# CycloneBoy/pdf_table

Hardware: AMD Instinct MI355X
Metric: pages/s (higher is better)
Workload: dtype bf16

## Files before the change

pdf_table_amd/csrc/det_kernels.hip:

```cpp
#include <math.h>

#include "common.h"

namespace PT_FMT_NS {

typedef __attribute__((ext_vector_type(4))) uint32_t u32x4;
typedef __attribute__((ext_vector_type(2))) uint32_t u32x2;

__device__ __forceinline__ float bf2f(uint32_t bits16) { return a16_to_f32(bits16); }
__device__ __forceinline__ uint32_t f2bf(float f) { return f32_to_a16(f); }

struct ResizeCoef {
  int s0, s1;
  int a0, a1;
};
__device__ __forceinline__ ResizeCoef resize_coef(int d, double scale, int ssize, bool clamp_frac) {
  float f = (float)(((double)d + 0.5) * scale - 0.5);
  int s = (int)floorf(f);
  f -= (float)s;
  ResizeCoef c;
  if (clamp_frac) {
    if (s < 0) { f = 0.f; s = 0; }
    if (s >= ssize - 1) { f = 0.f; s = ssize - 1; }
  }
// ... 43 lines not shown
      const int y = blockIdx.y * PRE_ROWS + ry;
      if (y >= nh) break;
      const long long i = ((long long)b * nh + y) * nw + x;
      int v[3];
      if (w == nw && h == nh) {
        const uint8_t* p = src + ((size_t)y * w + x) * 3;
        v[0] = p[0]; v[1] = p[1]; v[2] = p[2];
      } else if (area2) {
        const uint8_t* p0 = src + ((size_t)(2 * y) * w + 2 * x) * 3;
        const uint8_t* p1 = p0 + (size_t)w * 3;
#pragma unroll
        for (int c = 0; c < 3; ++c) v[c] = (p0[c] + p0[3 + c] + p1[c] + p1[3 + c] + 2) >> 2;
      } else {
        const ResizeCoef cy = resize_coef(y, sy, h, false);
        const uint8_t* r0 = src + (size_t)cy.s0 * w * 3;
        const uint8_t* r1 = src + (size_t)cy.s1 * w * 3;
        unsigned long long q0, q1;
        if (o0 + 8 <= w * 3) {
          __builtin_memcpy(&q0, r0 + o0, 8);
          __builtin_memcpy(&q1, r1 + o0, 8);
        } else {
          q0 = q1 = 0;
          for (int k = 0; k < 3; ++k) {
            q0 |= (unsigned long long)r0[o0 + k] << (8 * k) | (unsigned long long)r0[cx.s1 * 3 + k] << (d1 + 8 * k);
            q1 |= (unsigned long long)r1[o0 + k] << (8 * k) | (unsigned long long)r1[cx.s1 * 3 + k] << (d1 + 8 * k);
          }
        }
#pragma unroll
        for (int c = 0; c < 3; ++c) {
          const int S0 = (int)((q0 >> (8 * c)) & 0xFF) * cx.a0 + (int)((q0 >> (d1 + 8 * c)) & 0xFF) * cx.a1;
          const int S1 = (int)((q1 >> (8 * c)) & 0xFF) * cx.a0 + (int)((q1 >> (d1 + 8 * c)) & 0xFF) * cx.a1;
          v[c] = (((cy.a0 * (S0 >> 4)) >> 16) + ((cy.a1 * (S1 >> 4)) >> 16) + 2) >> 2;
          v[c] = v[c] < 0 ? 0 : (v[c] > 255 ? 255 : v[c]);
        }
      }
      const uint32_t e0 = lut[0][v[2]], e1 = lut[1][v[1]], e2 = lut[2][v[0]];
      if (!split) {
        u32x2 pk;
        pk.x = (e0 & 0xFFFFu) | (e1 << 16);
        pk.y = e2 & 0xFFFFu;
        *reinterpret_cast<u32x2*>(out + (size_t)i * 4) = pk;
      } else {
        u32x4 pk;
        pk.x = (e0 & 0xFFFFu) | (e1 << 16);
        pk.y = e2 & 0xFFFFu;
        pk.z = (e0 >> 16) | (e1 & 0xFFFF0000u);
        pk.w = e2 >> 16;
        *reinterpret_cast<u32x4*>(out + (size_t)i * 8) = pk;
      }
    }
  }
}

int pt_launch_det_preprocess(const uint8_t* pages, int n, int h, int w, int nh, int nw, int flavour, int split,
                             bf16_t* out, hipStream_t s) {
  PT_REQUIRE(n > 0 && nh > 0 && nw > 0 && nh < 65536 && n < 65536, "det pre-process: bad extents %d x %d x %d", n, nh, nw);
  hipLaunchKernelGGL(det_preprocess_kernel, dim3((nw + 255) / 256, (nh + PRE_ROWS - 1) / PRE_ROWS, n), dim3(256), 0, s, pages, n, h, w, nh, nw, flavour, split, out,
                     (double)w / nw, (double)h / nh);
  PT_HIP_CHECK(hipGetLastError());
  return PT_OK;
}

__device__ __forceinline__ uint32_t bfmax2(uint32_t a, uint32_t b) {
  const float al = a16lo_f32(a), bl = a16lo_f32(b);
  const float ah = a16hi_f32(a), bh = a16hi_f32(b);
  const uint32_t lo = (bl > al) ? (b & 0xFFFFu) : (a & 0xFFFFu);
  const uint32_t hi = (bh > ah) ? (b & 0xFFFF0000u) : (a & 0xFFFF0000u);
  return lo | hi;
}

__global__ __launch_bounds__(256) void maxpool3x3s2_split_kernel(const bf16_t* __restrict__ in, int B, int H, int W,
                                                                  int C, bf16_t* __restrict__ out) {
  a16_kernel_enter();
  const int Ho = (H + 2 - 3) / 2 + 1, Wo = (W + 2 - 3) / 2 + 1;
  const int cg = C >> 3;
  const long long total = (long long)B * Ho * Wo * cg;
  for (long long i = (long long)blockIdx.x * blockDim.x + threadIdx.x; i < total; i += (long long)gridDim.x * blockDim.x) {
    const int g = (int)(i % cg);
    long long t = i / cg;
    const int ox = (int)(t % Wo);
    t /= Wo;
    const int oy = (int)(t % Ho);
    const int b = (int)(t / Ho);
    uint32_t bh[8], bl[8];
    float bv[8];
    bool first = true;
    for (int dy = 0; dy < 3; ++dy) {
      const int iy = oy * 2 - 1 + dy;
      if ((unsigned)iy >= (unsigned)H) continue;
      for (int dx = 0; dx < 3; ++dx) {
        const int ix = ox * 2 - 1 + dx;
        if ((unsigned)ix >= (unsigned)W) continue;
        const bf16_t* px = in + (((size_t)b * H + iy) * W + ix) * (2 * C) + g * 8;
        const u32x4 vh = *reinterpret_cast<const u32x4*>(px);
        const u32x4 vl = *reinterpret_cast<const u32x4*>(px + C);
        const uint32_t hw[4] = {vh.x, vh.y, vh.z, vh.w}, lw[4] = {vl.x, vl.y, vl.z, vl.w};
#pragma unroll
        for (int k = 0; k < 8; ++k) {
          const uint32_t hb = (k & 1) ? (hw[k >> 1] >> 16) : (hw[k >> 1] & 0xFFFFu);
          const uint32_t lb = (k & 1) ? (lw[k >> 1] >> 16) : (lw[k >> 1] & 0xFFFFu);
          const float v = bf2f(hb) + bf2f(lb);
          if (first || v > bv[k]) { bv[k] = v; bh[k] = hb; bl[k] = lb; }
        }
        first = false;
      }
    }
    u32x4 oh, ol;
    oh.x = bh[0] | (bh[1] << 16); oh.y = bh[2] | (bh[3] << 16); oh.z = bh[4] | (bh[5] << 16); oh.w = bh[6] | (bh[7] << 16);
    ol.x = bl[0] | (bl[1] << 16); ol.y = bl[2] | (bl[3] << 16); ol.z = bl[4] | (bl[5] << 16); ol.w = bl[6] | (bl[7] << 16);
// ... 465 lines not shown
```

pdf_table_amd/csrc/lore_kernels.hip:

```cpp
#include <stdio.h>
#include <stdlib.h>

#include "common.h"

namespace PT_FMT_NS {

typedef __attribute__((ext_vector_type(4))) uint32_t u32x4;
typedef __attribute__((ext_vector_type(2))) uint32_t u32x2;

namespace {

__device__ __forceinline__ float bf2f(uint32_t b) { return a16_to_f32(b); }
__device__ __forceinline__ uint32_t f2bf(float f) { return f32_to_a16(f); }

__device__ __forceinline__ void load8(const bf16_t* p, int lo_off, int split, float* v) {
  const u32x4 h = *reinterpret_cast<const u32x4*>(p);
  const uint32_t hw[4] = {h.x, h.y, h.z, h.w};
#pragma unroll
  for (int k = 0; k < 8; ++k) v[k] = bf2f((k & 1) ? (hw[k >> 1] >> 16) : (hw[k >> 1] & 0xFFFFu));
  if (split) {
    const u32x4 l = *reinterpret_cast<const u32x4*>(p + lo_off);
    const uint32_t lw[4] = {l.x, l.y, l.z, l.w};
#pragma unroll
    for (int k = 0; k < 8; ++k) v[k] += bf2f((k & 1) ? (lw[k >> 1] >> 16) : (lw[k >> 1] & 0xFFFFu));
// ... 230 lines not shown
        else
          store8(out + oo, C, PACKED == 1 ? 0 : split, acc);
      }
  }
}

__global__ __launch_bounds__(256) void tsr_preprocess_kernel(const uint8_t* __restrict__ pages, int ph, int pw,
                                                              const pt_tsr_table* __restrict__ tabs, int H, int W, int bgr,
                                                              const float* __restrict__ lut, bf16_t* __restrict__ out,
                                                              int split) {
  a16_kernel_enter();
  const int t = blockIdx.y;
  const int i = blockIdx.x * blockDim.x + threadIdx.x;
  if (i >= H * W) return;
  const int y = i / W, x = i - y * W;
  const pt_tsr_table tb = tabs[t];
  auto sat = [](double v) { return (long long)fmin(fmax(rint(v), -2147483648.0), 2147483647.0); };
  const long long adelta = sat(tb.minv[0] * x * 1024.0), bdelta = sat(tb.minv[3] * x * 1024.0);
  const long long X0 = sat((tb.minv[1] * y + tb.minv[2]) * 1024.0) + 16, Y0 = sat((tb.minv[4] * y + tb.minv[5]) * 1024.0) + 16;
  const long long X = (X0 + adelta) >> 5, Y = (Y0 + bdelta) >> 5;
  long long sx = X >> 5, sy = Y >> 5;
  sx = sx < -32768 ? -32768 : (sx > 32767 ? 32767 : sx);
  sy = sy < -32768 ? -32768 : (sy > 32767 ? 32767 : sy);
  const int ax = (int)(X & 31), ay = (int)(Y & 31);
  const int wt[4] = {(32 - ay) * (32 - ax) * 32, (32 - ay) * ax * 32, ay * (32 - ax) * 32, ay * ax * 32};
  int acc[3] = {0, 0, 0};
  const uint8_t* pg = pages + (size_t)tb.page * ph * pw * 3;
#pragma unroll
  for (int k = 0; k < 4; ++k) {
    const long long yy = sy + (k >> 1), xx = sx + (k & 1);
    if (yy < 0 || yy >= tb.crop_h || xx < 0 || xx >= tb.crop_w) continue;
    const long long py = tb.y0 + yy, px = tb.x0 + xx;
    if (py < 0 || py >= ph || px < 0 || px >= pw) continue;
    const uint8_t* s = pg + ((size_t)py * pw + px) * 3;
    acc[0] += s[0] * wt[k]; acc[1] += s[1] * wt[k]; acc[2] += s[2] * wt[k];
  }
  float v[3];
#pragma unroll
  for (int c = 0; c < 3; ++c) {
    const int sc = bgr ? 2 - c : c;
    int u = (acc[sc] + (1 << 14)) >> 15;
    u = u < 0 ? 0 : (u > 255 ? 255 : u);
    v[c] = lut[c * 256 + u];
  }
  bf16_t* o = out + ((size_t)t * H * W + i) * (split ? 8 : 4);
  uint32_t hb[3];
#pragma unroll
  for (int c = 0; c < 3; ++c) { hb[c] = f2bf(v[c]); o[c] = (bf16_t)hb[c]; }
  o[3] = 0;
  if (split) {
#pragma unroll
    for (int c = 0; c < 3; ++c) o[4 + c] = (bf16_t)f2bf(v[c] - bf2f(hb[c]));
    o[7] = 0;
  }
}

typedef __attribute__((ext_vector_type(8))) __bf16 dbf16x8;
typedef __attribute__((ext_vector_type(16))) float df32x16;
typedef __attribute__((ext_vector_type(2))) float df2;
__device__ __forceinline__ uint32_t pack_df2(df2 v) { return pack_a16x2(v.x, v.y); }
__device__ __forceinline__ df2 unpack_df2(uint32_t pk) { return df2{a16lo_f32(pk), a16hi_f32(pk)}; }

template <int SPLIT, int NB>
__global__ __launch_bounds__(256, (SPLIT || NB > 64) ? 2 : 4) void dcn_fused_kernel(const bf16_t* __restrict__ x, const float* __restrict__ om,
                                                            const bf16_t* __restrict__ w, const float* __restrict__ bias,
                                                            bf16_t* __restrict__ out, long long npix, int H, int W, int C,
                                                            int N, int relu) {
#pragma clang fp contract(fast)
  a16_kernel_enter();
  constexpr int ROW = 80;
  constexpr int NP = SPLIT ? 2 : 1;
  constexpr int NT = NB / 32;
  __shared__ __attribute__((aligned(16))) char s_a[NP][128 * ROW];
  __shared__ __attribute__((aligned(16))) char s_w[NP][NB * ROW];
  const int tid = threadIdx.x, lane = tid & 63, wave = tid >> 6;
  const int lx = lane & 31, q = lane >> 5;
  const long long p0 = (long long)blockIdx.x * 128;
  const int n0 = blockIdx.y * NB;
  const int cs = SPLIT ? 2 * C : C;
  const int nslice = C >> 5, nk = 9 * nslice;
  const int gp = tid & 127, gh = tid >> 7;
  long long pix = p0 + gp;
  const bool live = pix < npix;
  if (!live) pix = npix - 1;
  const int xw = (int)(pix % W), yh = (int)((pix / W) % H);
  const bf16_t* xb = x + (size_t)(pix / ((long long)W * H)) * H * W * cs;
  const float* omp = om + pix * 32;
  constexpr int WPIECES = NB * 4 / 256;
  const bf16_t* wbase = w + (size_t)(n0 >> 6) * (SPLIT ? 3 : 1) * nk * (64 * 32);

  df32x16 acc[NT];
#pragma unroll
  for (int t = 0; t < NT; ++t)
#pragma unroll
    for (int r = 0; r < 16; ++r) acc[t][r] = 0.f;

  int coff[4];
  float cwt[4], mask = 0.f;
  u32x4 rc[NP][4][2];
  u32x4 rw[NP][WPIECES];

  auto geometry = [&](int tap) {
    const float off_h = omp[2 * tap], off_w = omp[2 * tap + 1];
    mask = 1.f / (1.f + expf(-omp[18 + tap]));
    const float h_im = (float)(yh - 1 + tap / 3) + off_h;
    const float w_im = (float)(xw - 1 + tap % 3) + off_w;
// ... 1399 lines not shown
  PT_HIP_CHECK(hipGetLastError());
  return PT_OK;
}

int pt_launch_dwconvt_up_add(const bf16_t* in, const float* w, const bf16_t* add, bf16_t* out, int B, int h, int wd,
                             int C, int f, int split, hipStream_t s) {
  PT_REQUIRE(in && w && out && C % 8 == 0 && (f == 2 || f == 4), "dwconvT: bad arguments");
  const long long blocks2 = (long long)B * h * wd * (C / 8);
  const char* sw = getenv("PT_DWCONVT2");
  if (f == 2 && blocks2 < (1ll << 31) && C <= 512 && !(sw && sw[0] == '0')) {
    static int packed = -1;
    if (packed < 0) {
      const char* ev = getenv("PT_DWCONVT2_PACKED");
      packed = ev ? atoi(ev) : 1;
    }
    if (!split && packed)
      hipLaunchKernelGGL(dwconvt_up2_add_kernel<1>, dim3(grid_for(blocks2)), dim3(256), (size_t)16 * C * sizeof(float), s, in, w, add, out,
                         B, h, wd, C, 0);
    else if (split && packed)
      hipLaunchKernelGGL(dwconvt_up2_add_kernel<2>, dim3(grid_for(blocks2)), dim3(256), (size_t)16 * C * sizeof(float), s, in, w, add, out,
                         B, h, wd, C, 1);
    else
      hipLaunchKernelGGL(dwconvt_up2_add_kernel<0>, dim3(grid_for(blocks2)), dim3(256), (size_t)16 * C * sizeof(float), s, in, w, add, out,
                         B, h, wd, C, split);
    PT_HIP_CHECK(hipGetLastError());
    return PT_OK;
  }
  hipLaunchKernelGGL(dwconvt_up_add_kernel, dim3(grid_for((long long)B * h * f * wd * f * (C / 8))), dim3(256), 0, s, in,
                     w, add, out, B, h, wd, C, f, split);
  PT_HIP_CHECK(hipGetLastError());
  return PT_OK;
}

int pt_launch_dwconvt_up2_slice(const bf16_t* in, const float* w, bf16_t* out, int out_cstride, int out_coff, int out_lo_off, int B,
                                int h, int wd, int C, int split, hipStream_t s) {
  PT_REQUIRE(in && w && out && C % 8 == 0 && C <= 512 && out_cstride % 8 == 0 && out_coff % 8 == 0 && out_lo_off % 8 == 0 &&
                 out_coff + C * (split ? 2 : 1) <= out_cstride && (!split || out_coff + out_lo_off + C <= out_cstride),
             "dwconvT slice: bad arguments");
  const long long blocks2 = (long long)B * h * wd * (C / 8);
  PT_REQUIRE(blocks2 < (1ll << 31), "dwconvT slice: map too large");
  if (split)
    hipLaunchKernelGGL((dwconvt_up2_add_kernel<2, true>), dim3(grid_for(blocks2)), dim3(256), (size_t)16 * C * sizeof(float), s, in, w,
                       (const bf16_t*)nullptr, out + out_coff, B, h, wd, C, 1, out_cstride, out_lo_off);
  else
    hipLaunchKernelGGL((dwconvt_up2_add_kernel<1, true>), dim3(grid_for(blocks2)), dim3(256), (size_t)16 * C * sizeof(float), s, in, w,
                       (const bf16_t*)nullptr, out + out_coff, B, h, wd, C, 0, out_cstride, 0);
  PT_HIP_CHECK(hipGetLastError());
  return PT_OK;
}

int pt_launch_tsr_preprocess(const uint8_t* pages, int ph, int pw, const pt_tsr_table* tabs, int n, int H, int W, int bgr,
                             const float* lut, bf16_t* out, int split, hipStream_t s) {
  PT_REQUIRE(pages && tabs && lut && out && n > 0 && H > 0 && W > 0, "tsr preprocess: bad arguments");
  hipLaunchKernelGGL(tsr_preprocess_kernel, dim3((H * W + 255) / 256, n), dim3(256), 0, s, pages, ph, pw, tabs, H, W, bgr, lut,
                     out, split);
  PT_HIP_CHECK(hipGetLastError());
  return PT_OK;
}

template <int SPLIT, int NB>
static int launch_dcn_fused(pt_engine* e, const bf16_t* x, const float* om, const bf16_t* w, const float* bias, bf16_t* out,
                            int B, int H, int W, int C, int N, int relu, hipStream_t s) {
  const long long npix = (long long)B * H * W;
  char label[48];
  snprintf(label, sizeof(label), "dcn fused %d->%d @%dx%d%s", C, N, H, W, SPLIT ? " x3" : "");
  PtProfScope prof(e, s, PT_PROF_OTHER, 0, label);
  hipLaunchKernelGGL((dcn_fused_kernel<SPLIT, NB>), dim3((unsigned)((npix + 127) / 128), N / NB), dim3(256), 0, s, x, om, w,
                     bias, out, npix, H, W, C, N, relu);
  PT_HIP_CHECK(hipGetLastError());
  return PT_OK;
}

bool pt_dcn_fuses_om(const pt_engine* e, int C, int split) {
  const char* ev = getenv("PT_DCN_FUSE_OM");
  const int on = ev ? atoi(ev) : 1;
  const char* nt = getenv("PT_DCN_THREADS");
  const char* ea = getenv("PT_DCN_EARLY");
  const char* xf = getenv("PT_DCN_X3_FAST");
  const bool defaults = !(nt && atoi(nt) != 512) && !(ea && atoi(ea) == 0) && !(xf && atoi(xf) == 0);
  if (!on || !e || C % 64 != 0 || !defaults || (!split && e->dcn_mfma != 0)) return false;
  return on == 2 || (!split && C <= 128);
}

bool pt_dcn_fuses_up(const pt_engine* e, int C, int N, int split) {
  const char* ev = getenv("PT_IDA_FUSE_UP");
  if ((ev && atoi(ev) == 0) || !e || split || e->dcn_mfma != 0 || C != N || (N != 64 && N != 128)) return false;
  for (const char* name : {"PT_DCN_FUSED", "PT_DCN_FUSE_OM", "PT_DCN_THREADS", "PT_DCN_EARLY", "PT_DCN_NB", "PT_DCN_MFMA", "PT_DCN_MFMA_NB", "PT_DCN_X3_FAST"})
    if (getenv(name)) return false;
  return true;
}

int pt_launch_dcn_fused(pt_engine* e, const bf16_t* x, const float* om, const bf16_t* w, const float* bias, bf16_t* out,
                        int B, int H, int W, int C, int N, int split, int relu, hipStream_t s, const bf16_t* omw, const float* omb,
                        const bf16_t* up_in, const float* up_w, int up_f) {
  PT_REQUIRE(e && x && (om || (omw && omb)) && w && bias && out && C % 32 == 0 && N % 64 == 0, "dcn fused: bad arguments (C=%d N=%d)", C, N);
  PT_REQUIRE(!omw || pt_dcn_fuses_om(e, C, split), "dcn fused: the offset conv can only be fused on the default fused64 paths (C=%d)", C);
  PT_REQUIRE((long long)H * W * (split ? 2 * C : C) < (1ll << 31), "dcn fused: image too large for 32-bit offsets");
  if (up_f) {
    PT_REQUIRE(up_in && up_w && (up_f == 2 || (up_f == 4 && N == 64)) && H % up_f == 0 && W % up_f == 0,
               "dcn fused + up: factor %d must be 2 (or 4 at 64 channels) and divide the %dx%d map", up_f, H, W);
    PT_REQUIRE(pt_dcn_fuses_up(e, C, N, split), "dcn fused + up: only the default single-pass kernels at C = N = 64 or 128 carry the up-sampling epilogue (C=%d N=%d split=%d)", C, N, split);
  }
  const double dcn_bytes = (double)B * H * W * ((split ? 2.0 : 1.0) * 2.0 * (C + N) + 27 * 4.0) + (double)N * 9 * C * 2.0 * (split ? 3 : 1) +
                           (up_f ? (double)B * (H / up_f) * (W / up_f) * N * 2.0 : 0.0);
  e->prof.next_bytes = dcn_bytes;
  static int x3fast = -1;
// ... 152 lines not shown
```

pdf_table_amd/csrc/rec_kernels.hip:

```cpp
#include <math.h>

#include "common.h"

namespace PT_FMT_NS {

typedef __attribute__((ext_vector_type(8))) __bf16 bf16x8;
typedef __attribute__((ext_vector_type(16))) float f32x16;
typedef __attribute__((ext_vector_type(4))) uint32_t u32x4;
typedef __attribute__((ext_vector_type(2))) uint32_t u32x2;

__device__ __forceinline__ float rbf2f(uint32_t bits16) { return a16_to_f32(bits16); }
__device__ __forceinline__ uint32_t rf2bf(float f) { return f32_to_a16(f); }

__global__ __launch_bounds__(256) void rec_warp_kernel(const uint8_t* __restrict__ pages, int ph, int pw,
                                                        const pt_rec_line* __restrict__ lines, int n_lines,
                                                        const long long* __restrict__ pix_off, uint8_t* __restrict__ crops) {
  a16_kernel_enter();
  const int li = blockIdx.y;
  if (li >= n_lines) return;
  const pt_rec_line L = lines[li];
  const int cw = L.crop_w, chh = L.crop_h;
  const long long npx = (long long)cw * chh;
  uint8_t* dst = crops + pix_off[li] * 3;
  const uint8_t* src = pages + (size_t)L.page * ph * pw * 3;
  for (long long i = (long long)blockIdx.x * blockDim.x + threadIdx.x; i < npx; i += (long long)gridDim.x * blockDim.x) {
    const int x = (int)(i % cw), y = (int)(i / cw);
    int v[3];
    pt_warp_sample(src, ph, pw, L.minv, x, y, v);
#pragma unroll
    for (int c = 0; c < 3; ++c) dst[i * 3 + c] = (uint8_t)v[c];
  }
}

__global__ __launch_bounds__(1024) void rec_offsets_kernel(const pt_rec_line* __restrict__ lines, int n,
                                                           long long* __restrict__ off) {
  a16_kernel_enter();
  __shared__ long long sc[1024];
  __shared__ long long carry;
  const int tid = threadIdx.x;
  if (tid == 0) { carry = 0; off[0] = 0; }
  __syncthreads();
  for (int base = 0; base < n; base += 1024) {
    const int i = base + tid;
    long long v = 0;
    if (i < n) {
      v = (long long)lines[i].crop_w * (long long)lines[i].crop_h;
      if (v < 0) v = 0;
    }
    sc[tid] = v;
    __syncthreads();
    for (int d = 1; d < 1024; d <<= 1) {
      const long long t = tid >= d ? sc[tid - d] : 0;
      __syncthreads();
      sc[tid] += t;
      __syncthreads();
    }
    if (i < n) off[i + 1] = carry + sc[tid];
    __syncthreads();
    if (tid == 1023) carry += sc[1023];
    __syncthreads();
  }
}

int pt_launch_rec_offsets(const pt_rec_line* lines, int n, long long* off, hipStream_t s) {
  hipLaunchKernelGGL(rec_offsets_kernel, dim3(1), dim3(1024), 0, s, lines, n, off);
  PT_HIP_CHECK(hipGetLastError());
  return PT_OK;
}

int pt_launch_rec_warp(const uint8_t* pages, int ph, int pw, const pt_rec_line* lines, int n_lines,
                       const long long* pix_off, uint8_t* crops, int max_crop_px, hipStream_t s) {
  if (n_lines <= 0) return PT_OK;
  int bx = (max_crop_px + 255) / 256;
  bx = bx < 1 ? 1 : (bx > 64 ? 64 : bx);
  hipLaunchKernelGGL(rec_warp_kernel, dim3(bx, n_lines), dim3(256), 0, s, pages, ph, pw, lines, n_lines, pix_off, crops);
  PT_HIP_CHECK(hipGetLastError());
  return PT_OK;
}

struct RCoef {
  int s0, s1, a0, a1;
};
__device__ __forceinline__ RCoef rcoef(int d, double scale, int ssize, bool clamp_frac) {
  float f = (float)(((double)d + 0.5) * scale - 0.5);
  int s = (int)floorf(f);
  f -= (float)s;
  if (clamp_frac) {
    if (s < 0) { f = 0.f; s = 0; }
    if (s >= ssize - 1) { f = 0.f; s = ssize - 1; }
  }
  RCoef c;
  c.a0 = (int)rintf((1.f - f) * 2048.f);
  c.a1 = (int)rintf(f * 2048.f);
  int t0 = s, t1 = s + 1;
  c.s0 = t0 < 0 ? 0 : (t0 >= ssize ? ssize - 1 : t0);
  c.s1 = t1 < 0 ? 0 : (t1 >= ssize ? ssize - 1 : t1);
  return c;
}

__global__ __launch_bounds__(256) void rec_resize_gray_kernel(const uint8_t* __restrict__ crops,
                                                               const pt_rec_line* __restrict__ lines,
                                                               const long long* __restrict__ pix_off, int n_lines, int TH,
                                                               int TWID, int split, bf16_t* __restrict__ out,
                                                               float* __restrict__ out_f32) {
  a16_kernel_enter();
  const long long total = (long long)n_lines * TH * TWID;
  for (long long i = (long long)blockIdx.x * blockDim.x + threadIdx.x; i < total; i += (long long)gridDim.x * blockDim.x) {
    const int x = (int)(i % TWID);
    const long long t = i / TWID;
    const int y = (int)(t % TH);
    const int li = (int)(t / TH);
    const int cw = lines[li].crop_w, chh = lines[li].crop_h;
    float gray = 0.f;
    if (cw > 0 && chh > 0) {
      const double ratio = (double)cw / (double)chh;
      const int nw = ratio > (double)TWID / (double)TH ? TWID : (int)((double)TH * ratio);
      if (x < nw) {
        const uint8_t* src = crops + pix_off[li] * 3;
        int v[3];
        if (cw == nw && chh == TH) {
          const uint8_t* p = src + ((size_t)y * cw + x) * 3;
          v[0] = p[0]; v[1] = p[1]; v[2] = p[2];
        } else if (cw == 2 * nw && chh == 2 * TH) {
          const uint8_t* p0 = src + ((size_t)(2 * y) * cw + 2 * x) * 3;
          const uint8_t* p1 = p0 + (size_t)cw * 3;
#pragma unroll
          for (int c = 0; c < 3; ++c) v[c] = (p0[c] + p0[3 + c] + p1[c] + p1[3 + c] + 2) >> 2;
        } else {
          const RCoef cx = rcoef(x, (double)cw / nw, cw, true);
          const RCoef cy = rcoef(y, (double)chh / TH, chh, false);
          const uint8_t* r0 = src + (size_t)cy.s0 * cw * 3;
          const uint8_t* r1 = src + (size_t)cy.s1 * cw * 3;
#pragma unroll
          for (int c = 0; c < 3; ++c) {
            const int S0 = r0[cx.s0 * 3 + c] * cx.a0 + r0[cx.s1 * 3 + c] * cx.a1;
            const int S1 = r1[cx.s0 * 3 + c] * cx.a0 + r1[cx.s1 * 3 + c] * cx.a1;
            int r = (((cy.a0 * (S0 >> 4)) >> 16) + ((cy.a1 * (S1 >> 4)) >> 16) + 2) >> 2;
            v[c] = r < 0 ? 0 : (r > 255 ? 255 : r);
          }
        }
        const float R = (float)v[0] / 255.f, G = (float)v[1] / 255.f, B = (float)v[2] / 255.f;
        gray = (R * 0.2989f + G * 0.5870f) + B * 0.1140f;
      }
    }
    if (out_f32) {
      out_f32[i] = gray;
      continue;
    }
    const uint32_t hb = rf2bf(gray);
    if (split) {
      out[i * 2] = (bf16_t)hb;
      out[i * 2 + 1] = (bf16_t)rf2bf(gray - rbf2f(hb));
    } else {
      out[i] = (bf16_t)hb;
    }
  }
}

int pt_launch_rec_resize_gray(const uint8_t* crops, const pt_rec_line* lines, const long long* pix_off, int n_lines,
                              int split, bf16_t* out, hipStream_t s) {
  if (n_lines <= 0) return PT_OK;
  const long long total = (long long)n_lines * 32 * 640;
  int blocks = (int)((total + 255) / 256);
  if (blocks > 256 * 32) blocks = 256 * 32;
  hipLaunchKernelGGL(rec_resize_gray_kernel, dim3(blocks), dim3(256), 0, s, crops, lines, pix_off, n_lines, 32, 640, split, out,
                     static_cast<float*>(nullptr));
  PT_HIP_CHECK(hipGetLastError());
  return PT_OK;
}

int pt_launch_rec_resize_gray_f32(const uint8_t* crops, const pt_rec_line* lines, const long long* pix_off, int n_lines, int tw,
                                  float* out, hipStream_t s) {
  if (n_lines <= 0) return PT_OK;
  const long long total = (long long)n_lines * 32 * tw;
  int blocks = (int)((total + 255) / 256);
  if (blocks > 256 * 32) blocks = 256 * 32;
  hipLaunchKernelGGL(rec_resize_gray_kernel, dim3(blocks), dim3(256), 0, s, crops, lines, pix_off, n_lines, 32, tw, 0,
                     static_cast<bf16_t*>(nullptr), out);
  PT_HIP_CHECK(hipGetLastError());
  return PT_OK;
}

__global__ void crnn_limits_kernel(const pt_rec_line* __restrict__ lines, int n, int* l1, int* l2a, int* l2b, int* l3a, int* l3b,
                                   int* l0, int* __restrict__ cols) {
  a16_kernel_enter();
  __shared__ int sums[6];
  if (threadIdx.x < 6) sums[threadIdx.x] = 0;
  __syncthreads();
  int acc[6] = {0, 0, 0, 0, 0, 0};
  for (int b = blockIdx.x * blockDim.x + threadIdx.x; b < n; b += gridDim.x * blockDim.x) {
    const int cw = lines[b].crop_w, chh = lines[b].crop_h;
    int nw = 0;
    if (cw > 0 && chh > 0) {
      const double ratio = (double)cw / (double)chh;
      nw = ratio > 640.0 / 32.0 ? 640 : (int)(32.0 * ratio);
    }
    const int e0 = (nw + 2) >> 1;
    const int e1 = (e0 + 2) >> 1;
    const int v[5] = {min(e0 + 1, 320), min(e1 + 1, 160), min(e1 + 2, 160), min(e1 + 3, 160), min(e1 + 4, 160)};
    l1[b] = v[0]; l2a[b] = v[1]; l2b[b] = v[2]; l3a[b] = v[3]; l3b[b] = v[4];
    l0[b] = min((v[0] + 31) / 32 * 32 + 1, 320);
    const int tw[5] = {32, 32, 32, 32, 32}, wo[5] = {320, 160, 160, 160, 160};
#pragma unroll
    for (int k = 0; k < 5; ++k) acc[k] += min(wo[k], (v[k] + tw[k] - 1) / tw[k] * tw[k]);
    acc[5] += min(160, (v[4] + 31) / 32 * 32);
  }
#pragma unroll
  for (int k = 0; k < 6; ++k) atomicAdd(&sums[k], acc[k]);
  __syncthreads();
  if (threadIdx.x < 6) atomicAdd(&cols[threadIdx.x], sums[threadIdx.x]);
}

__global__ __launch_bounds__(1024) void rows_live_list_kernel(const int* __restrict__ lim, int n, int* __restrict__ glist) {
  a16_kernel_enter();
  __shared__ int part[1024];
  const int tid = threadIdx.x, per = (n + 1023) / 1024, b0 = tid * per, b1 = min(n, b0 + per);
  int cnt = 0;
  for (int b = b0; b < b1; ++b) cnt += min(PT_REC_T / 32, (lim[b] + 31) / 32);
  part[tid] = cnt;
  __syncthreads();
  for (int off = 1; off < 1024; off <<= 1) {
    const int v = tid >= off ? part[tid - off] : 0;
    __syncthreads();
    part[tid] += v;
    __syncthreads();
  }
// ... 1856 lines not shown
```

Measured before the change: 815.3.

## Add fast preprocessing kernels for detection, TSR, rec warp and resize

Adds four new preprocessing kernels, each on by default and switchable through a PT_PRE_FAST environment variable. Detection resize batches row loads and reuses horizontal passes across rows. TSR warp caches the LUT and per-row transforms in shared memory. Rec warp switches to a flat grid over all crop pixels using binary search on the offsets, and rec resize-gray uses one block per line with per-column coefficients in shared memory and vectorized stores. These target memory traffic and load imbalance in the preprocessing stages, at the risk of small numeric differences and extra code paths.

```diff
diff --git a/pdf_table_amd/csrc/det_kernels.hip b/pdf_table_amd/csrc/det_kernels.hip
--- a/pdf_table_amd/csrc/det_kernels.hip
+++ b/pdf_table_amd/csrc/det_kernels.hip
@@ -119,9 +119,127 @@
   }
 }
 
+constexpr int PRE_FAST_ROWS = 16, PRE_FAST_BATCH = 8;
+
+__global__ __launch_bounds__(256) void det_preprocess_fast_kernel(const uint8_t* __restrict__ pages, int n, int h, int w,
+                                                                   int nh, int nw, int flavour, int split, bf16_t* __restrict__ out,
+                                                                   double sx, double sy) {
+  a16_kernel_enter();
+  __shared__ uint32_t lut[3][256];
+  __shared__ int rowc[PRE_FAST_ROWS][4];
+  {
+    const int u = threadIdx.x;
+#pragma unroll
+    for (int c = 0; c < 3; ++c) {
+      float o;
+      if (flavour == PT_DET_PRE_DB_TORCH) {
+        const float mean[3] = {123.68f, 116.78f, 103.94f};
+        o = ((float)u - mean[c]) / 255.f;
+      } else {
+        const float scale = (float)(1.0 / 255.0);
+        const float mean[3] = {0.485f, 0.456f, 0.406f};
+        const float stdv[3] = {0.229f, 0.224f, 0.225f};
+        o = ((float)u * scale - mean[c]) / stdv[c];
+      }
+      const uint32_t hi = f2bf(o);
+      lut[c][u] = hi | (f2bf(o - bf2f(hi)) << 16);
+    }
+    if (u < PRE_FAST_ROWS) {
+      const int y = min((int)blockIdx.y * PRE_FAST_ROWS + u, nh - 1);
+      const ResizeCoef cy = resize_coef(y, sy, h, false);
+      rowc[u][0] = cy.s0; rowc[u][1] = cy.s1; rowc[u][2] = cy.a0; rowc[u][3] = cy.a1;
+    }
+  }
+  __syncthreads();
+  const int x = blockIdx.x * blockDim.x + threadIdx.x;
+  if (x >= nw) return;
+  const int b = blockIdx.z;
+  const uint8_t* src = pages + (size_t)b * h * w * 3;
+  const ResizeCoef cx = resize_coef(x, sx, w, true);
+  const int o0 = cx.s0 * 3, d1 = (cx.s1 - cx.s0) * 24;
+  const bool wide = o0 + 8 <= w * 3;
+  auto bytes = [&](int row) {
+    const uint8_t* r = src + (size_t)row * w * 3;
+    unsigned long long q = 0;
+    for (int k = 0; k < 3; ++k) q |= (unsigned long long)r[o0 + k] << (8 * k) | (unsigned long long)r[cx.s1 * 3 + k] << (d1 + 8 * k);
+    return q;
+  };
+  auto hpass = [&](unsigned long long q, int S[3]) {
+    const uint32_t p0 = (uint32_t)q, p1 = d1 ? (uint32_t)(q >> 24) : p0;
+#pragma unroll
+    for (int c = 0; c < 3; ++c) S[c] = (__mul24((int)((p0 >> (8 * c)) & 0xFF), cx.a0) + __mul24((int)((p1 >> (8 * c)) & 0xFF), cx.a1)) >> 4;
+  };
+  int have = -1;
+  int H1[3] = {0, 0, 0};
+  for (int g = 0; g < PRE_FAST_ROWS; g += PRE_FAST_BATCH) {
+    if ((int)blockIdx.y * PRE_FAST_ROWS + g >= nh) break;
+    unsigned long long q0[PRE_FAST_BATCH], q1[PRE_FAST_BATCH];
+    int s0[PRE_FAST_BATCH], s1[PRE_FAST_BATCH];
+#pragma unroll
+    for (int k = 0; k < PRE_FAST_BATCH; ++k) {
+      s0[k] = __builtin_amdgcn_readfirstlane(rowc[g + k][0]);
+      s1[k] = __builtin_amdgcn_readfirstlane(rowc[g + k][1]);
+      q0[k] = q1[k] = 0;
+      if (s0[k] != (k ? s1[k - 1] : have)) {
+        if (wide) __builtin_memcpy(&q0[k], src + (size_t)s0[k] * w * 3 + o0, 8); else q0[k] = bytes(s0[k]);
+      }
+      if (s1[k] != s0[k]) {
+        if (wide) __builtin_memcpy(&q1[k], src + (size_t)s1[k] * w * 3 + o0, 8); else q1[k] = bytes(s1[k]);
+      }
+    }
+#pragma unroll
+    for (int k = 0; k < PRE_FAST_BATCH; ++k) {
+      const int y = (int)blockIdx.y * PRE_FAST_ROWS + g + k;
+      if (y >= nh) break;
+      const int a0 = __builtin_amdgcn_readfirstlane(rowc[g + k][2]), a1 = __builtin_amdgcn_readfirstlane(rowc[g + k][3]);
+      int H0[3];
+      if (s0[k] != (k ? s1[k - 1] : have)) {
+        hpass(q0[k], H0);
+      } else {
+        H0[0] = H1[0]; H0[1] = H1[1]; H0[2] = H1[2];
+      }
+      if (s1[k] != s0[k]) {
+        hpass(q1[k], H1);
+      } else {
+        H1[0] = H0[0]; H1[1] = H0[1]; H1[2] = H0[2];
+      }
+      int v[3];
+#pragma unroll
+      for (int c = 0; c < 3; ++c) {
+        v[c] = ((__mul24(a0, H0[c]) >> 16) + (__mul24(a1, H1[c]) >> 16) + 2) >> 2;
+        v[c] = v[c] < 0 ? 0 : (v[c] > 255 ? 255 : v[c]);
+      }
+      const long long i = ((long long)b * nh + y) * nw + x;
+      const uint32_t e0 = lut[0][v[2]], e1 = lut[1][v[1]], e2 = lut[2][v[0]];
+      if (!split) {
+        u32x2 pk;
+        pk.x = (e0 & 0xFFFFu) | (e1 << 16);
+        pk.y = e2 & 0xFFFFu;
+        *reinterpret_cast<u32x2*>(out + (size_t)i * 4) = pk;
+      } else {
+        u32x4 pk;
+        pk.x = (e0 & 0xFFFFu) | (e1 << 16);
+        pk.y = e2 & 0xFFFFu;
+        pk.z = (e0 >> 16) | (e1 & 0xFFFF0000u);
+        pk.w = e2 >> 16;
+        *reinterpret_cast<u32x4*>(out + (size_t)i * 8) = pk;
+      }
+    }
+    have = s1[PRE_FAST_BATCH - 1];
+  }
+}
+
 int pt_launch_det_preprocess(const uint8_t* pages, int n, int h, int w, int nh, int nw, int flavour, int split,
                              bf16_t* out, hipStream_t s) {
   PT_REQUIRE(n > 0 && nh > 0 && nw > 0 && nh < 65536 && n < 65536, "det pre-process: bad extents %d x %d x %d", n, nh, nw);
+  const char* sw = getenv("PT_PRE_FAST");
+  const bool resample = !(w == nw && h == nh) && !(w == 2 * nw && h == 2 * nh);
+  if (resample && !(sw && sw[0] == '0')) {
+    hipLaunchKernelGGL(det_preprocess_fast_kernel, dim3((nw + 255) / 256, (nh + PRE_FAST_ROWS - 1) / PRE_FAST_ROWS, n), dim3(256), 0, s, pages, n, h, w, nh,
+                       nw, flavour, split, out, (double)w / nw, (double)h / nh);
+    PT_HIP_CHECK(hipGetLastError());
+    return PT_OK;
+  }
   hipLaunchKernelGGL(det_preprocess_kernel, dim3((nw + 255) / 256, (nh + PRE_ROWS - 1) / PRE_ROWS, n), dim3(256), 0, s, pages, n, h, w, nh, nw, flavour, split, out,
                      (double)w / nw, (double)h / nh);
   PT_HIP_CHECK(hipGetLastError());
diff --git a/pdf_table_amd/csrc/lore_kernels.hip b/pdf_table_amd/csrc/lore_kernels.hip
--- a/pdf_table_amd/csrc/lore_kernels.hip
+++ b/pdf_table_amd/csrc/lore_kernels.hip
@@ -306,6 +306,100 @@
 #pragma unroll
     for (int c = 0; c < 3; ++c) o[4 + c] = (bf16_t)f2bf(v[c] - bf2f(hb[c]));
     o[7] = 0;
+  }
+}
+
+constexpr int TSR_TILE_H = 32, TSR_BATCH = 4;
+__global__ __launch_bounds__(256) void tsr_preprocess_fast_kernel(const uint8_t* __restrict__ pages, int ph, int pw,
+                                                                   const pt_tsr_table* __restrict__ tabs, int H, int W, int bgr,
+                                                                   const float* __restrict__ lut, bf16_t* __restrict__ out,
+                                                                   int split) {
+  a16_kernel_enter();
+  __shared__ uint32_t slut[3 * 256];
+  __shared__ long long rowt[TSR_TILE_H][2];
+  const int tid = threadIdx.x, t = blockIdx.z;
+  const pt_tsr_table tb = tabs[t];
+  auto sat = [](double v) { return (long long)fmin(fmax(rint(v), -2147483648.0), 2147483647.0); };
+  for (int k = tid; k < 3 * 256; k += 256) {
+    const float v = lut[k];
+    const uint32_t hb = f2bf(v);
+    slut[k] = hb | (f2bf(v - bf2f(hb)) << 16);
+  }
+  const int yb = blockIdx.y * TSR_TILE_H;
+  if (tid < TSR_TILE_H) {
+    const int y = yb + tid;
+    rowt[tid][0] = sat((tb.minv[1] * y + tb.minv[2]) * 1024.0) + 16;
+    rowt[tid][1] = sat((tb.minv[4] * y + tb.minv[5]) * 1024.0) + 16;
+  }
+  __syncthreads();
+  const int x = blockIdx.x * 64 + (tid & 63);
+  if (x >= W) return;
+  const long long adelta = sat(tb.minv[0] * x * 1024.0), bdelta = sat(tb.minv[3] * x * 1024.0);
+  const uint8_t* pg = pages + (size_t)tb.page * ph * pw * 3;
+  auto bound = [](long long v) { return (int)(v < -65536 ? -65536 : (v > 65536 ? 65536 : v)); };
+  const int xlo = bound(tb.x0 < 0 ? -(long long)tb.x0 : 0), xhi = bound((long long)pw - tb.x0 < tb.crop_w ? (long long)pw - tb.x0 : tb.crop_w);
+  const int ylo = bound(tb.y0 < 0 ? -(long long)tb.y0 : 0), yhi = bound((long long)ph - tb.y0 < tb.crop_h ? (long long)ph - tb.y0 : tb.crop_h);
+  const int last = ph * pw - 1;
+  for (int r0 = tid >> 6; r0 < TSR_TILE_H; r0 += 4 * TSR_BATCH) {
+    if (yb + r0 >= H) break;
+    uint32_t q[TSR_BATCH][4];
+    int wt[TSR_BATCH][4];
+#pragma unroll
+    for (int k = 0; k < TSR_BATCH; ++k) {
+      const int r = r0 + 4 * k;
+      const int X = (int)((rowt[r][0] + adelta) >> 5), Y = (int)((rowt[r][1] + bdelta) >> 5);
+      int sx = X >> 5, sy = Y >> 5;
+      sx = sx < -32768 ? -32768 : (sx > 32767 ? 32767 : sx);
+      sy = sy < -32768 ? -32768 : (sy > 32767 ? 32767 : sy);
+      const int ax = X & 31, ay = Y & 31;
+      const int w4[4] = {__mul24(32 - ay, 32 - ax) * 32, __mul24(32 - ay, ax) * 32, __mul24(ay, 32 - ax) * 32, __mul24(ay, ax) * 32};
+#pragma unroll
+      for (int j = 0; j < 4; ++j) {
+        const int yy = sy + (j >> 1), xx = sx + (j & 1);
+        wt[k][j] = (yy >= ylo && yy < yhi && xx >= xlo && xx < xhi) ? w4[j] : 0;
+        const long long pyl = (long long)tb.y0 + yy, pxl = (long long)tb.x0 + xx;
+        const int py = (int)(pyl < 0 ? 0 : (pyl > ph - 1 ? ph - 1 : pyl)), px = (int)(pxl < 0 ? 0 : (pxl > pw - 1 ? pw - 1 : pxl));
+        const int pi = __mul24(py, pw) + px;
+        const int adj = pi == last ? 1 : 0;
+        uint32_t v;
+        __builtin_memcpy(&v, pg + (pi * 3 - adj), 4);
+        q[k][j] = v >> (8 * adj);
+      }
+    }
+#pragma unroll
+    for (int k = 0; k < TSR_BATCH; ++k) {
+      const int y = yb + r0 + 4 * k;
+      if (y >= H) break;
+      int acc[3] = {0, 0, 0};
+#pragma unroll
+      for (int j = 0; j < 4; ++j) {
+        acc[0] += __mul24((int)(q[k][j] & 0xFF), wt[k][j]);
+        acc[1] += __mul24((int)((q[k][j] >> 8) & 0xFF), wt[k][j]);
+        acc[2] += __mul24((int)((q[k][j] >> 16) & 0xFF), wt[k][j]);
+      }
+      uint32_t e[3];
+#pragma unroll
+      for (int c = 0; c < 3; ++c) {
+        const int sc = bgr ? 2 - c : c;
+        int u = (acc[sc] + (1 << 14)) >> 15;
+        u = u < 0 ? 0 : (u > 255 ? 255 : u);
+        e[c] = slut[c * 256 + u];
+      }
+      const size_t i = (size_t)t * H * W + (size_t)y * W + x;
+      if (!split) {
+        u32x2 pk;
+        pk.x = (e[0] & 0xFFFFu) | (e[1] << 16);
+        pk.y = e[2] & 0xFFFFu;
+        *reinterpret_cast<u32x2*>(out + i * 4) = pk;
+      } else {
+        u32x4 pk;
+        pk.x = (e[0] & 0xFFFFu) | (e[1] << 16);
+        pk.y = e[2] & 0xFFFFu;
+        pk.z = (e[0] >> 16) | (e[1] & 0xFFFF0000u);
+        pk.w = e[2] >> 16;
+        *reinterpret_cast<u32x4*>(out + i * 8) = pk;
+      }
+    }
   }
 }
 
@@ -1811,6 +1905,14 @@
 int pt_launch_tsr_preprocess(const uint8_t* pages, int ph, int pw, const pt_tsr_table* tabs, int n, int H, int W, int bgr,
                              const float* lut, bf16_t* out, int split, hipStream_t s) {
   PT_REQUIRE(pages && tabs && lut && out && n > 0 && H > 0 && W > 0, "tsr preprocess: bad arguments");
+  const char* sw = getenv("PT_PRE_FAST");
+  if (!(sw && sw[0] == '0') && n < 65536 && (H + TSR_TILE_H - 1) / TSR_TILE_H < 65536 && ph > 0 && pw > 0 && ph < (1 << 23) && pw < (1 << 23) && (long long)ph * pw >= 2 &&
+      (long long)ph * pw * 3 < (1ll << 31)) {
+    hipLaunchKernelGGL(tsr_preprocess_fast_kernel, dim3((W + 63) / 64, (H + TSR_TILE_H - 1) / TSR_TILE_H, n), dim3(256), 0, s, pages, ph, pw, tabs, H, W,
+                       bgr, lut, out, split);
+    PT_HIP_CHECK(hipGetLastError());
+    return PT_OK;
+  }
   hipLaunchKernelGGL(tsr_preprocess_kernel, dim3((H * W + 255) / 256, n), dim3(256), 0, s, pages, ph, pw, tabs, H, W, bgr, lut,
                      out, split);
   PT_HIP_CHECK(hipGetLastError());
diff --git a/pdf_table_amd/csrc/rec_kernels.hip b/pdf_table_amd/csrc/rec_kernels.hip
--- a/pdf_table_amd/csrc/rec_kernels.hip
+++ b/pdf_table_amd/csrc/rec_kernels.hip
@@ -32,6 +32,87 @@
   }
 }
 
+__device__ __forceinline__ void warp_sample32(const uint8_t* __restrict__ src, int ph, int pw, const double* m, bool use_winv, double winv, int x, int y,
+                                              int v[3]) {
+  const double X0 = m[0] * x + m[1] * y + m[2];
+  const double Y0 = m[3] * x + m[4] * y + m[5];
+  double W = winv;
+  if (!use_winv) {
+    W = m[6] * x + m[7] * y + m[8];
+    W = W != 0. ? 32. / W : 0.;
+  }
+  const double fX = fmax(-2147483648., fmin(2147483647., X0 * W));
+  const double fY = fmax(-2147483648., fmin(2147483647., Y0 * W));
+  const int Xi = (int)rint(fX), Yi = (int)rint(fY);
+  const int sx = Xi >> 5, sy = Yi >> 5;
+  const int ax = Xi & 31, ay = Yi & 31;
+  const int w00 = __mul24(32 - ay, 32 - ax) * 32, w01 = __mul24(32 - ay, ax) * 32, w10 = __mul24(ay, 32 - ax) * 32, w11 = __mul24(ay, ax) * 32;
+  int acc[3] = {0, 0, 0};
+  auto tap = [&](int yy, int xx, int wgt) {
+    if (wgt && yy >= 0 && yy < ph && xx >= 0 && xx < pw) {
+      const uint8_t* p = src + ((size_t)yy * pw + xx) * 3;
+      acc[0] += __mul24(p[0], wgt); acc[1] += __mul24(p[1], wgt); acc[2] += __mul24(p[2], wgt);
+    }
+  };
+  tap(sy, sx, w00); tap(sy, sx + 1, w01); tap(sy + 1, sx, w10); tap(sy + 1, sx + 1, w11);
+#pragma unroll
+  for (int c = 0; c < 3; ++c) {
+    const int t = (acc[c] + (1 << 14)) >> 15;
+    v[c] = t < 0 ? 0 : (t > 255 ? 255 : t);
+  }
+}
+
+constexpr int WARP_FLAT_BLOCKS = 2048;
+
+__global__ __launch_bounds__(256) void rec_warp_fast_kernel(const uint8_t* __restrict__ pages, int ph, int pw,
+                                                             const pt_rec_line* __restrict__ lines, int n_lines,
+                                                             const long long* __restrict__ pix_off, uint8_t* __restrict__ crops) {
+  a16_kernel_enter();
+  const long long total = pix_off[n_lines];
+  long long chunk = (total + gridDim.x - 1) / gridDim.x;
+  chunk = (chunk + 255) & ~255ll;
+  const long long beg = (long long)blockIdx.x * chunk;
+  const long long end = beg + chunk < total ? beg + chunk : total;
+  long long p = beg + threadIdx.x;
+  if (p >= end) return;
+  int li = 0;
+  for (int hi = n_lines; hi - li > 1;) {
+    const int mid = (li + hi) >> 1;
+    if (pix_off[mid] <= p) li = mid; else hi = mid;
+  }
+  while (p < end) {
+    while (pix_off[li + 1] <= p) ++li;
+    const long long base = pix_off[li], next = pix_off[li + 1];
+    const long long stop = next < end ? next : end;
+    const pt_rec_line L = lines[li];
+    const int cw = L.crop_w;
+    const uint8_t* src = pages + (size_t)L.page * ph * pw * 3;
+    const bool use_winv = L.minv[6] == 0. && L.minv[7] == 0.;
+    const double winv = L.minv[8] != 0. ? 32. / L.minv[8] : 0.;
+    if (next - base > 0x7FFFFFFFll || cw <= 0) {
+      for (; p < stop; p += 256) {
+        const long long i = p - base;
+        int v[3];
+        warp_sample32(src, ph, pw, L.minv, use_winv, winv, (int)(i % cw), (int)(i / cw), v);
+        uint8_t* o = crops + p * 3;
+        o[0] = (uint8_t)v[0]; o[1] = (uint8_t)v[1]; o[2] = (uint8_t)v[2];
+      }
+      continue;
+    }
+    const uint32_t ucw = (uint32_t)cw, i0 = (uint32_t)(p - base);
+    const uint32_t dy = 256u / ucw, dx = 256u - dy * ucw;
+    uint32_t y = i0 / ucw, x = i0 - y * ucw;
+    for (; p < stop; p += 256) {
+      int v[3];
+      warp_sample32(src, ph, pw, L.minv, use_winv, winv, (int)x, (int)y, v);
+      uint8_t* o = crops + p * 3;
+      o[0] = (uint8_t)v[0]; o[1] = (uint8_t)v[1]; o[2] = (uint8_t)v[2];
+      x += dx; y += dy;
+      if (x >= ucw) { x -= ucw; ++y; }
+    }
+  }
+}
+
 __global__ __launch_bounds__(1024) void rec_offsets_kernel(const pt_rec_line* __restrict__ lines, int n,
                                                            long long* __restrict__ off) {
   a16_kernel_enter();
@@ -68,12 +149,20 @@
   return PT_OK;
 }
 
+static bool pre_fast() {
+  const char* sw = getenv("PT_PRE_FAST");
+  return !(sw && sw[0] == '0');
+}
+
 int pt_launch_rec_warp(const uint8_t* pages, int ph, int pw, const pt_rec_line* lines, int n_lines,
                        const long long* pix_off, uint8_t* crops, int max_crop_px, hipStream_t s) {
   if (n_lines <= 0) return PT_OK;
   int bx = (max_crop_px + 255) / 256;
   bx = bx < 1 ? 1 : (bx > 64 ? 64 : bx);
-  hipLaunchKernelGGL(rec_warp_kernel, dim3(bx, n_lines), dim3(256), 0, s, pages, ph, pw, lines, n_lines, pix_off, crops);
+  if (pre_fast())
+    hipLaunchKernelGGL(rec_warp_fast_kernel, dim3(WARP_FLAT_BLOCKS), dim3(256), 0, s, pages, ph, pw, lines, n_lines, pix_off, crops);
+  else
+    hipLaunchKernelGGL(rec_warp_kernel,dim3(bx, n_lines), dim3(256), 0, s, pages, ph, pw, lines, n_lines, pix_off, crops);
   PT_HIP_CHECK(hipGetLastError());
   return PT_OK;
 }
@@ -157,9 +246,120 @@
   }
 }
 
+constexpr int RG_ROWS = 16, RG_MAXW = 1024;
+
+__global__ __launch_bounds__(256) void rec_resize_gray_fast_kernel(const uint8_t* __restrict__ crops,
+                                                                    const pt_rec_line* __restrict__ lines,
+                                                                    const long long* __restrict__ pix_off, int n_lines, int TH,
+                                                                    int TWID, int split, bf16_t* __restrict__ out,
+                                                                    float* __restrict__ out_f32) {
+  a16_kernel_enter();
+  __shared__ float q255[256];
+  __shared__ int cxs[RG_MAXW];
+  __shared__ uint32_t cxa[RG_MAXW];
+  __shared__ int cys[RG_ROWS][4];
+  const int tid = threadIdx.x, li = blockIdx.x;
+  const int yb = blockIdx.y * RG_ROWS, rows = min(RG_ROWS, TH - yb);
+  const int cw = lines[li].crop_w, chh = lines[li].crop_h;
+  q255[tid] = (float)tid / 255.f;
+  int nw = 0;
+  if (cw > 0 && chh > 0) {
+    const double ratio = (double)cw / (double)chh;
+    nw = ratio > (double)TWID / (double)TH ? TWID : (int)((double)TH * ratio);
+    nw = nw < TWID ? nw : TWID;
+  }
+  const int mode = nw <= 0 ? 0 : (cw == nw && chh == TH) ? 1 : (cw == 2 * nw && chh == 2 * TH) ? 2 : 3;
+  if (mode == 3) {
+    for (int x = tid; x < nw; x += 256) {
+      const RCoef c = rcoef(x, (double)cw / nw, cw, true);
+      cxs[x] = c.s0 * 3;
+      cxa[x] = (uint32_t)c.a0 | ((uint32_t)c.a1 << 16) | (c.s1 != c.s0 ? 0x80000000u : 0u);
+    }
+    if (tid < rows) {
+      const RCoef c = rcoef(yb + tid, (double)chh / TH, chh, false);
+      cys[tid][0] = c.s0; cys[tid][1] = c.s1; cys[tid][2] = c.a0; cys[tid][3] = c.a1;
+    }
+  }
+  __syncthreads();
+  const uint8_t* src = crops + pix_off[li] * 3;
+  const int nq = TWID >> 2;
+  for (int g = tid; g < rows * nq; g += 256) {
+    const int r = g / nq, x0 = (g - r * nq) * 4, y = yb + r;
+    float gray[4] = {0.f, 0.f, 0.f, 0.f};
+    if (x0 < nw) {
+      const uint8_t *r0 = src, *r1 = src;
+      int a0 = 0, a1 = 0;
+      if (mode == 3) {
+        r0 = src + (size_t)cys[r][0] * cw * 3;
+        r1 = src + (size_t)cys[r][1] * cw * 3;
+        a0 = cys[r][2]; a1 = cys[r][3];
+      }
+#pragma unroll
+      for (int j = 0; j < 4; ++j) {
+        const int x = x0 + j;
+        if (x >= nw) break;
+        int v[3];
+        if (mode == 1) {
+          const uint8_t* p = src + ((size_t)y * cw + x) * 3;
+          v[0] = p[0]; v[1] = p[1]; v[2] = p[2];
+        } else if (mode == 2) {
+          const uint8_t* p0 = src + ((size_t)(2 * y) * cw + 2 * x) * 3;
+          const uint8_t* p1 = p0 + (size_t)cw * 3;
+#pragma unroll
+          for (int c = 0; c < 3; ++c) v[c] = (p0[c] + p0[3 + c] + p1[c] + p1[3 + c] + 2) >> 2;
+        } else {
+          const int o0 = cxs[x];
+          const uint32_t pa = cxa[x];
+          const int o1 = o0 + ((pa >> 31) ? 3 : 0), b0 = (int)(pa & 0xFFFFu), b1 = (int)((pa >> 16) & 0x7FFFu);
+#pragma unroll
+          for (int c = 0; c < 3; ++c) {
+            const int S0 = __mul24(r0[o0 + c], b0) + __mul24(r0[o1 + c], b1);
+            const int S1 = __mul24(r1[o0 + c], b0) + __mul24(r1[o1 + c], b1);
+            const int t = ((__mul24(a0, S0 >> 4) >> 16) + (__mul24(a1, S1 >> 4) >> 16) + 2) >> 2;
+            v[c] = t < 0 ? 0 : (t > 255 ? 255 : t);
+          }
+        }
+        const float R = q255[v[0]], G = q255[v[1]], B = q255[v[2]];
+        gray[j] = (R * 0.2989f + G * 0.5870f) + B * 0.1140f;
+      }
+    }
+    const size_t i = ((size_t)li * TH + y) * TWID + x0;
+    if (out_f32) {
+      *reinterpret_cast<float4*>(out_f32 + i) = make_float4(gray[0], gray[1], gray[2], gray[3]);
+      continue;
+    }
+    uint32_t hb[4];
+#pragma unroll
+    for (int j = 0; j < 4; ++j) hb[j] = rf2bf(gray[j]);
+    if (split) {
+      u32x4 pk;
+      pk.x = hb[0] | (rf2bf(gray[0] - rbf2f(hb[0])) << 16);
+      pk.y = hb[1] | (rf2bf(gray[1] - rbf2f(hb[1])) << 16);
+      pk.z = hb[2] | (rf2bf(gray[2] - rbf2f(hb[2])) << 16);
+      pk.w = hb[3] | (rf2bf(gray[3] - rbf2f(hb[3])) << 16);
+      *reinterpret_cast<u32x4*>(out + i * 2) = pk;
+    } else {
+      u32x2 pk;
+      pk.x = hb[0] | (hb[1] << 16);
+      pk.y = hb[2] | (hb[3] << 16);
+      *reinterpret_cast<u32x2*>(out + i) = pk;
+    }
+  }
+}
+
+static bool rg_fast_ok(int tw, const void* out, size_t align) {
+  return pre_fast() && tw % 4 == 0 && tw <= RG_MAXW && (reinterpret_cast<uintptr_t>(out) & (align - 1)) == 0;
+}
+
 int pt_launch_rec_resize_gray(const uint8_t* crops, const pt_rec_line* lines, const long long* pix_off, int n_lines,
                               int split, bf16_t* out, hipStream_t s) {
   if (n_lines <= 0) return PT_OK;
+  if (rg_fast_ok(640, out, split ? 16 : 8)) {
+    hipLaunchKernelGGL(rec_resize_gray_fast_kernel, dim3(n_lines, 32 / RG_ROWS), dim3(256), 0, s, crops, lines, pix_off, n_lines, 32, 640, split, out,
+                       static_cast<float*>(nullptr));
+    PT_HIP_CHECK(hipGetLastError());
+    return PT_OK;
+  }
   const long long total = (long long)n_lines * 32 * 640;
   int blocks = (int)((total + 255) / 256);
   if (blocks > 256 * 32) blocks = 256 * 32;
@@ -172,6 +372,12 @@
 int pt_launch_rec_resize_gray_f32(const uint8_t* crops, const pt_rec_line* lines, const long long* pix_off, int n_lines, int tw,
                                   float* out, hipStream_t s) {
   if (n_lines <= 0) return PT_OK;
+  if (rg_fast_ok(tw, out, 16)) {
+    hipLaunchKernelGGL(rec_resize_gray_fast_kernel, dim3(n_lines, 32 / RG_ROWS), dim3(256), 0, s, crops, lines, pix_off, n_lines, 32, tw, 0,
+                       static_cast<bf16_t*>(nullptr), out);
+    PT_HIP_CHECK(hipGetLastError());
+    return PT_OK;
+  }
   const long long total = (long long)n_lines * 32 * tw;
   int blocks = (int)((total + 255) / 256);
   if (blocks > 256 * 32) blocks = 256 * 32;
```

Result: no change. 822.8 (median of 6 runs) (+0.9%).
